# WLBF/flex-gpu-scheduler

Hardware: AMD Instinct MI355X
Metric: pods/sec sched throughput + p99 PodGroup gang-admit latency, 1/2/4/8-GPU groups (higher is better)
Workload: dtype int64

## Files before the change

### csrc/common/strings.h

```cpp
#pragma once

#include <cctype>
#include <string_view>

namespace xsched {

inline std::string_view trim(std::string_view s) {
  while (!s.empty() && std::isspace(static_cast<unsigned char>(s.front()))) s.remove_prefix(1);
  while (!s.empty() && std::isspace(static_cast<unsigned char>(s.back()))) s.remove_suffix(1);
  return s;
}

}
```

### csrc/framework/framework.cc

```cpp
#include "framework/framework.h"

#include <algorithm>
#include <atomic>
#include <stdexcept>

#include "scheduler/metrics.h"
#include "scheduler/queue.h"

namespace xsched {

namespace {
const std::pair<const char*, uint32_t> kPointNames[] = {
    {"queueSort", kQueueSort}, {"preFilter", kPreFilter}, {"filter", kFilter},   {"postFilter", kPostFilter},
    {"preScore", kPreScore},   {"score", kScore},         {"reserve", kReserve}, {"permit", kPermit},
    {"preBind", kPreBind},     {"bind", kBind},           {"postBind", kPostBind},
};
}

const char* ext_point_name(uint32_t p) {
  for (const auto& kv : kPointNames)
    if (kv.second == p) return kv.first;
  return "unknown";
}

// ... 569 lines not shown
    if (skip[k]) skipped_total += scorers_[k].first->score_skip_value() * scorers_[k].second;
  if (plain_mask) {
    for (size_t i = 0; i < n; ++i) total[i].score += skipped_total + plain_tot[i];
  } else if (skipped_total) {
    for (size_t i = 0; i < n; ++i) total[i].score += skipped_total;
  }
  for (size_t k = 0; k < scorers_.size(); ++k) {
    if (skip[k] || is_plain(k)) continue;
    auto& pl = scorers_[k].first;
    if (pl->has_normalize_score()) {
      if (pl->normalize_uses_names())
        for (size_t i = 0; i < n; ++i) per[k][i].name = &nodes[i]->name();
      Status st = pl->normalize_score(s, p, per[k]);
      if (!st.is_success()) return Status(Code::Error, "running Normalize on Score plugin " + pl->name() + ": " + st.message());
    }
    int64_t w = scorers_[k].second;
    if (breakdown) {
      std::vector<int64_t> v(n);
      for (size_t i = 0; i < n; ++i) v[i] = per[k][i].score;
      breakdown->emplace_back(pl->name() + "*" + std::to_string(w), std::move(v));
    }
    for (size_t i = 0; i < n; ++i) {
      int64_t sc = per[k][i].score;
      if (sc > kMaxNodeScore || sc < kMinNodeScore)
        return Status(Code::Error, "plugin \"" + pl->name() + "\" returns an invalid score " + std::to_string(sc) +
                                       ", it should in the range of [0, 100] after normalizing");
      total[i].score += sc * w;
    }
  }
  record("Score", Status(), t0, s);
  return {};
}

Status Framework::run_reserve(CycleState& s, const PodPtr& p, const std::string& node) {
  auto it = chain_.find(kReserve);
  if (it == chain_.end()) return {};
  for (const auto& pl : it->second) {
    Status st = pl->reserve(s, p, node);
    if (!st.is_success()) {
      Status e(Code::Error, "running Reserve plugin \"" + pl->name() + "\": " + st.message());
      if (st.is_unschedulable()) e = Status(st.code(), st.message());
      e.with_plugin(pl->name_ptr());
      return e;
    }
  }
  return {};
}

void Framework::run_unreserve(CycleState& s, const PodPtr& p, const std::string& node) {
  auto it = chain_.find(kReserve);
  if (it == chain_.end()) return;
  for (auto rit = it->second.rbegin(); rit != it->second.rend(); ++rit) (*rit)->unreserve(s, p, node);
}

Status Framework::run_permit(CycleState& s, const PodPtr& p, const std::string& node,
                             std::function<void(const Status&)> on_done) {
  auto it = chain_.find(kPermit);
  if (it == chain_.end()) return {};
  constexpr size_t kInline = 4;
  WaitingPods::Timeout inline_timeouts[kInline];
  std::vector<WaitingPods::Timeout> more_timeouts;
  size_t nwait = 0;
  for (const auto& pl : it->second) {
    auto [st, timeout] = pl->permit(s, p, node);
    if (st.is_success()) continue;
    if (st.is_unschedulable()) {
// ... 84 lines not shown
```

### csrc/framework/framework.h

```cpp
#pragma once

#include <map>
#include <memory>
#include <string>
#include <unordered_map>
#include <vector>

#include "framework/plugin.h"
#include "framework/waiting_pods.h"

namespace xsched {

struct ProfileConfig {
  std::string scheduler_name = kDefaultSchedulerName;
  std::map<uint32_t, std::vector<std::string>> enabled;
  std::map<std::string, int64_t> score_weights;
  std::map<std::string, Json> plugin_args;
  int percentage_of_nodes_to_score = 0;
  bool run_all_filters = false;
  static ProfileConfig from_json(const Json& j);
};

struct EqTable {
  size_t n = 0;
// ... 42 lines not shown
class Framework {
 public:
  Framework(const ProfileConfig& cfg, Handle handle);
  ~Framework();

  const std::string& profile_name() const { return cfg_.scheduler_name; }
  const ProfileConfig& config() const { return cfg_; }
  Handle& handle() { return handle_; }
  PluginPtr plugin(const std::string& name) const;
  const std::vector<PluginPtr>& all_plugins() const { return all_; }
  bool has(uint32_t point) const;

  bool less(const QueuedPodInfo& a, const QueuedPodInfo& b) const;

  Status run_pre_filter(CycleState& s, const Pod& p);
  Status run_pre_filter_add_pod(CycleState& s, const Pod& to_schedule, const PodPtr& to_add, const NodeInfo& ni);
  Status run_pre_filter_remove_pod(CycleState& s, const Pod& to_schedule, const PodPtr& to_remove, const NodeInfo& ni);
  bool pre_filter_extensions_affected(const CycleState& s, const Pod& to_schedule, const Pod& other,
                                      const std::string* except = nullptr) const;
  Status run_filter(CycleState& s, const Pod& p, const NodeInfo& ni);
  Status run_filter_with_nominated_pods(CycleState& s, const Pod& p, const NodeInfo& ni);
  uint64_t nominated_signature(const CycleState& s, const Pod& p, const NodeInfo& ni, bool* cacheable) const;
  uint64_t nominated_signature(const CycleState& s, const Pod& p, const std::vector<PodPtr>* list,
                               bool* cacheable) const;
  Status run_filter_with_nominated_pods_inplace(CycleState& s, const Pod& p, NodeInfo& ni);
  std::pair<PostFilterResult, Status> run_post_filter(CycleState& s, const Pod& p, const NodeStatusMap& m);
  Status run_pre_score(CycleState& s, const Pod& p, const NodeList& nodes);
  using ScoreBreakdown = std::vector<std::pair<std::string, std::vector<int64_t>>>;
  Status run_score(CycleState& s, const Pod& p, const NodeList& nodes, std::vector<NodeScore>& total,
                   ScoreBreakdown* breakdown = nullptr, EqScoreCache* eq = nullptr);
  bool filters_node_local(const Pod& p, const Snapshot& s) const;
  std::vector<char> local_scorers(const Pod& p, const Snapshot& s) const;
  void local_scorers(const Pod& p, const Snapshot& s, std::vector<char>& out) const;
  Status run_reserve(CycleState& s, const PodPtr& p, const std::string& node);
  void run_unreserve(CycleState& s, const PodPtr& p, const std::string& node);
  Status run_permit(CycleState& s, const PodPtr& p, const std::string& node, std::function<void(const Status&)> on_done);
  Status run_pre_bind(CycleState& s, const PodPtr& p, const std::string& node);
  Status run_bind(CycleState& s, const PodPtr& p, const std::string& node);
  void run_post_bind(CycleState& s, const PodPtr& p, const std::string& node);

  std::vector<ClusterEvent> events_for(const std::string& plugin) const;
  std::vector<std::string> watched_kinds() const;
  void dispatch_object_event(const std::string& kind, int type, const JsonPtr& obj, const JsonPtr& old);
  void notify_capacity_freed();
  void start();
  void stop();

  static constexpr int64_t kMaxPermitTimeoutUs = 15LL * 60 * 1000000;

 private:
  Status filter_with_nominated(CycleState& s, const Pod& p, const NodeInfo& ni, NodeInfo* inplace);
  ParallelSite score_site_;
  void record(const char* point, const Status& st, int64_t start_us, CycleState& s);
  ProfileConfig cfg_;
  Handle handle_;
  std::vector<PluginPtr> all_;
  std::map<std::string, PluginPtr> by_name_;
  std::map<uint32_t, std::vector<PluginPtr>> chain_;
  std::vector<std::pair<PluginPtr, int64_t>> scorers_;
  std::unordered_map<std::string, std::vector<PluginPtr>> kind_watchers_;
  std::vector<PluginPtr> capacity_watchers_;
  PluginPtr queue_sort_;
};

}
```

### csrc/framework/plugin.h

```cpp
#pragma once

#include <functional>
#include <memory>
#include <string>
#include <unordered_map>
#include <utility>
#include <vector>

#include "common/clock.h"
#include "common/json.h"
#include "common/parallel.h"
#include "framework/types.h"

#define XS_FIXED_STATUS(code, msg)                                 \
  ([]() -> const ::xsched::Status& {                               \
    static const ::xsched::Status fixed_status = ::xsched::Status::immortal(code, msg); \
    return fixed_status;                                          \
  }())

namespace xsched {

class Framework;
class SchedulerCache;
class Informers;
// ... 64 lines not shown
  uint32_t points() const { return points_; }

  virtual bool less(const QueuedPodInfo& a, const QueuedPodInfo& b) const { return false; }
  virtual Status pre_filter(CycleState& s, const Pod& p) { return {}; }
  virtual bool has_pre_filter_extensions() const { return false; }
  virtual Status add_pod(CycleState& s, const Pod& to_schedule, const PodPtr& to_add, const NodeInfo& ni) {
    return {};
  }
  virtual Status remove_pod(CycleState& s, const Pod& to_schedule, const PodPtr& to_remove, const NodeInfo& ni) {
    return {};
  }
  virtual bool pre_filter_extension_affects(const CycleState& s, const Pod& to_schedule, const Pod& other) const {
    return true;
  }
  virtual Status filter(CycleState& s, const Pod& p, const NodeInfo& ni) { return {}; }
  virtual bool skip_filter(const Pod& p) const { return false; }
  virtual std::pair<PostFilterResult, Status> post_filter(CycleState& s, const Pod& p, const NodeStatusMap& m) {
    return {PostFilterResult{}, Status(Code::Unschedulable)};
  }
  virtual Status pre_score(CycleState& s, const Pod& p, const NodeList& nodes) { return {}; }
  virtual std::pair<int64_t, Status> score(CycleState& s, const Pod& p, const NodeInfo& ni) { return {0, {}}; }
  virtual Status score_many(CycleState& s, const Pod& p, const NodeList& nodes, const char* skip,
                            std::vector<NodeScore>& out, const int* pos = nullptr) {
    for (size_t i = 0; i < nodes.size(); ++i) {
      if (skip && skip[i]) continue;
      auto [sc, st] = score(s, p, *nodes[i]);
      if (!st.is_success()) return st;
      out[i].score = sc;
    }
    return {};
  }
  virtual bool has_normalize_score() const { return false; }
  virtual Status normalize_score(CycleState& s, const Pod& p, std::vector<NodeScore>& scores) { return {}; }
  virtual Status reserve(CycleState& s, const PodPtr& p, const std::string& node) { return {}; }
  virtual void unreserve(CycleState& s, const PodPtr& p, const std::string& node) {}
  virtual std::pair<Status, int64_t> permit(CycleState& s, const PodPtr& p, const std::string& node) {
    return {Status(), 0};
  }
  virtual Status pre_bind(CycleState& s, const PodPtr& p, const std::string& node) { return {}; }
  virtual Status bind(CycleState& s, const PodPtr& p, const std::string& node) { return Status(Code::Skip); }
  virtual void post_bind(CycleState& s, const PodPtr& p, const std::string& node) {}
  virtual bool filter_node_local(const Pod& p, const Snapshot& s) const { return false; }
  virtual bool score_node_local(const Pod& p, const Snapshot& s) const { return false; }
  virtual bool score_all_zero(const Pod& p, const Snapshot& s) const { return false; }
  virtual int64_t score_skip_value() const { return 0; }
  virtual bool normalize_uses_names() const { return false; }
  virtual std::vector<ClusterEvent> events_to_register() const { return {}; }
  virtual void on_object_event(const std::string& kind, int type, const JsonPtr& obj, const JsonPtr& old) {}
  virtual std::vector<std::string> watched_kinds() const { return {}; }
  virtual bool wants_capacity_events() const { return false; }
  virtual void capacity_freed() {}
  virtual void start() {}
  virtual void stop() {}
  virtual Json debug_call(const std::string& what, CycleState& s, const PodPtr& p, const Json& args) {
    Json out = Json::object();
    out.set("error", Json(name() + " has no debug call " + what));
    return out;
  }

 protected:
  std::string name_;
  const std::string* name_ptr_;
  uint32_t points_;
};
using PluginPtr = std::shared_ptr<Plugin>;

// ... 23 lines not shown
```

### csrc/plugins/flexgpu.cc

```cpp
#include <algorithm>
#include <cstdint>
#include <cstdio>
#include <string>

#include "common/log.h"
#include "framework/plugin.h"
#include "scheduler/cache.h"

namespace xsched {
namespace {

constexpr const char* kFlexGPUStateKey = "FlexGPU/assignment";

using Demand = GpuDemand;

struct Placement {
  std::vector<int> gpus;
  std::vector<std::pair<int, int>> parts;
  bool ok() const { return !gpus.empty(); }
  void clear() {
    gpus.clear();
    parts.clear();
  }
};

void place_whole(const GpuLedger& L, int64_t k, Placement& pl) {
  pl.clear();
  if (k <= 0) k = 1;
  int n_free = 0;
  for (int g = 0; g < L.gpu_count; ++g) n_free += L.whole_gpu_free(g);
  if (n_free < k) return;
  int best_numa = INT32_MIN, best_count = 0, distinct = 0, first_numa = INT32_MAX;
  for (int g = 0; g < L.gpu_count; ++g) {
    if (!L.whole_gpu_free(g)) continue;
    const int numa = L.numa[g];
    bool seen = false;
    for (int h = 0; h < g && !seen; ++h) seen = L.whole_gpu_free(h) && L.numa[h] == numa;
    if (seen) continue;
// ... 54 lines not shown
  bool best_breaks = true;
  for (int g = 0; g < L.gpu_count; ++g) {
    if (L.monopoly[g] > 0 || L.free[g].max_slot_mem < m) continue;
    int64_t cap = L.part_mem(g);
    bool breaks = L.whole_gpu_free(g);
    for (int p = 0; p < L.parts[g]; ++p) {
      const auto& s = L.slots[L.offset[g] + p];
      if (s.exclusive > 0 || s.fenced) continue;
      int64_t remain = cap - s.used_mem - m;
      if (remain < 0) continue;
      if (bg < 0 || (!breaks && best_breaks) || (breaks == best_breaks && remain < best_remain)) {
        bg = g;
        bp = p;
        best_remain = remain;
        best_breaks = breaks;
      }
    }
  }
  if (breaks_whole) *breaks_whole = bg >= 0 && best_breaks;
  if (bg < 0 || !build) return;
  pl.gpus.push_back(bg);
  pl.parts.emplace_back(bg, bp);
}

void place(const GpuLedger& L, const Demand& d, Placement& pl) {
  switch (d.kind) {
    case Demand::Gpu: return place_whole(L, d.amount, pl);
    case Demand::Xcd: return place_xcd(L, d.amount, pl);
    case Demand::Memory: return place_memory(L, d.amount, pl);
    default: pl.clear();
  }
}

void append_int(std::string& s, int v) {
  char buf[16];
  int n = std::snprintf(buf, sizeof buf, "%d", v);
  s.append(buf, static_cast<size_t>(n));
}

void join_ints(const std::vector<int>& v, std::string& s) {
  s.clear();
  for (size_t i = 0; i < v.size(); ++i) {
    if (i) s += ',';
    append_int(s, v[i]);
  }
}

void join_parts(const std::vector<std::pair<int, int>>& v, std::string& s) {
  s.clear();
  for (size_t i = 0; i < v.size(); ++i) {
    if (i) s += ',';
    append_int(s, v[i].first);
    s += ':';
    append_int(s, v[i].second);
  }
}

std::string join_ints(const std::vector<int>& v) {
  std::string s;
  join_ints(v, s);
  return s;
}

std::string join_parts(const std::vector<std::pair<int, int>>& v) {
  std::string s;
  join_parts(v, s);
  return s;
}

struct AssignmentState : StateData {
  std::string index, partitions;
  Json annotations(const GpuNames& gn) const {
    Json a = Json::object();
    a.set(gn.index_annotation, Json(index));
    if (!partitions.empty()) a.set(gn.partition_annotation, Json(partitions));
    return a;
  }
  std::shared_ptr<StateData> clone() const override { return std::make_shared<AssignmentState>(*this); }
};

class FlexGPU : public Plugin {
 public:
  bool filter_node_local(const Pod&, const Snapshot&) const override { return true; }
  bool score_node_local(const Pod&, const Snapshot&) const override { return true; }
  FlexGPU(const Json&, Handle& h) : Plugin("FlexGPU", kFilter | kScore | kReserve | kBind), h_(h), gn_(*h.gpu_names) {}

  Status filter(CycleState&, const Pod& p, const NodeInfo& ni) override {
    const Demand& d = p.gpu_demand;
    if (XS_V(6)) log_filter(p, ni);
    if (d.kind == Demand::None) return {};
    if (d.kind == Demand::Conflict) return Status::unresolvable("pod conflict resources");
    const GpuNames& gn = gn_;
    int gid = gn.gpu_id();
    int kid = d.kind == Demand::Gpu ? gid : d.kind == Demand::Xcd ? gn.xcd_id() : gn.memory_id();
    if (!ni.allocatable.has(gid) || !ni.allocatable.has(kid)) return Status::unresolvable("unknown resource type");
    if (ni.requested.get(kid) + d.amount > ni.allocatable.get(kid)) return failure(kid, false);
    if (!fits(ni.gpu, d)) return failure(kid, true);
    return {};
  }

  void log_filter(const Pod& p, const NodeInfo& ni) const {
    XS_LOGV(6, "pod info").kv("point", "filter").kv("pod", p.key()).kv("node", ni.name());
    for (const auto& c : p.containers)
      for (int id : {gn_.gpu_id(), gn_.xcd_id(), gn_.memory_id()})
// ... 38 lines not shown
        for (int g = 0; g < L.gpu_count; ++g)
          if (L.free[g].max_slot_mem >= d.amount) return true;
        return false;
      }
      default: return false;
    }
  }

  std::pair<int64_t, Status> score(CycleState&, const Pod& p, const NodeInfo& ni) override {
    const Demand& d = p.gpu_demand;
    switch (d.kind) {
      case Demand::Gpu: return {ni.gpu.free_gpus(), {}};
      case Demand::Xcd: {
        int waste = 0;
        Placement none;
        place_xcd(ni.gpu, d.amount, none, &waste, false);
        return {ni.gpu.free_xcds() + 64 * waste, {}};
      }
      case Demand::Memory: {
        bool breaks = false;
        Placement none;
        place_memory(ni.gpu, d.amount, none, &breaks, false);
        return {ni.gpu.free_memory() + (breaks ? 8 * ni.gpu.mem_per_gpu : 0), {}};
      }
      default: return {0, {}};
    }
  }
  bool has_normalize_score() const override { return true; }
  Status normalize_score(CycleState&, const Pod&, std::vector<NodeScore>& s) override {
    default_normalize_score(kMaxNodeScore, true, s);
    return {};
  }

  Status reserve(CycleState& s, const PodPtr& p, const std::string& node) override {
    const Demand& d = p->gpu_demand;
    if (d.kind == Demand::None) return {};
    if (d.kind == Demand::Conflict) return Status::unresolvable("pod conflict resources");
    NodeInfoPtr ni = h_.snapshot ? h_.snapshot->get(node) : nullptr;
    if (!ni) return Status::error("getting node \"" + node + "\" from Snapshot");
    thread_local Placement pl;
    place(ni->gpu, d, pl);
    if (!pl.ok()) return Status::unschedulable("allocate index fail");
    XS_LOGV(6, "assigned gpu indexes").kv("pod", p->key()).kv("node", node).kv("indexes", join_ints(pl.gpus))
        .kv("partitions", join_parts(pl.parts));
    const GpuNames& gn = gn_;
    auto st = s.reuse<AssignmentState>(kFlexGPUStateKey);
    join_ints(pl.gpus, st->index);
    join_parts(pl.parts, st->partitions);
    h_.cache->annotate_assumed_pod(p->uid(), [&](Pod& cp) {
      StrMap& am = cp.meta.annotations.mut();
      am.reserve(am.size() + 2);
      auto put = [&](const std::string& k, const std::string& v) {
        for (auto& a : am)
          if (a.first == k) {
            a.second = v;
            return;
          }
        am.emplace_back(k, v);
      };
      put(gn.index_annotation, st->index);
      if (!st->partitions.empty()) put(gn.partition_annotation, st->partitions);
      cp.set_gpu_assignment(pl.gpus, pl.parts, gn);
    }, false);
    s.write(kFlexGPUStateKey, st);
    return {};
  }

  void unreserve(CycleState& s, const PodPtr& p, const std::string&) override {
    const GpuNames& gn = gn_;
    s.erase(kFlexGPUStateKey);
    if (!h_.cache->is_assumed(p->uid())) return;
    h_.cache->mutate_pod(p->uid(), [&](Pod& cp) {
      auto& a = cp.meta.annotations.mut();
      a.erase(std::remove_if(a.begin(), a.end(),
                             [&](const auto& kv) {
                               return kv.first == gn.index_annotation || kv.first == gn.partition_annotation;
                             }),
              a.end());
    });
  }

  Status bind(CycleState& s, const PodPtr& p, const std::string& node) override {
    Json ann = Json::object();
    if (auto* st = s.read_as<AssignmentState>(kFlexGPUStateKey)) ann = st->annotations(gn_);
    try {
      h_.client->bind(*p, node, ann);
    } catch (const std::exception& e) {
      return Status::error(e.what());
    }
    return {};
  }

  std::vector<ClusterEvent> events_to_register() const override {
    return {{"Pod", kDelete, ""}, {"Node", kAdd | kUpdateNodeAllocatable | kUpdateNodeLabel, ""}};
  }

// ... 13 lines not shown
```

### csrc/scheduler/queue.cc

```cpp
#include "scheduler/queue.h"

#include <algorithm>
#include <chrono>

namespace xsched {

void PodHeap::swap_at(size_t a, size_t b) {
  std::swap(v_[a], v_[b]);
  v_[a]->heap_index = a;
  v_[b]->heap_index = b;
}

void PodHeap::up(size_t i) {
  while (i > 0) {
    size_t p = (i - 1) / 2;
    if (!less_(*v_[i], *v_[p])) break;
    swap_at(i, p);
    i = p;
  }
}

void PodHeap::down(size_t i) {
  size_t n = v_.size();
  for (;;) {
// ... 268 lines not shown
    if (mark == kActivate) {
      active_.push(p);
      activated = true;
    } else if (mark == kPark) {
      parked_[uid] = p;
    } else if (move_request_cycle_ >= pod_cycle) {
      backoff_.push(p);
    } else {
      unschedulable_[uid] = p;
    }
  }
  nominator_->add(p->pod, "");
  if (activated) cv_.notify_all();
  return true;
}

size_t SchedulingQueue::pending_activations() const {
  std::lock_guard<AdaptiveMutex> g(mu_);
  size_t n = 0;
  for (const auto& kv : in_flight_) n += kv.second == kActivate;
  return n;
}

size_t SchedulingQueue::in_flight() const {
  std::lock_guard<AdaptiveMutex> g(mu_);
  return in_flight_.size();
}

int64_t SchedulingQueue::scheduling_cycle() const {
  std::lock_guard<AdaptiveMutex> g(mu_);
  return scheduling_cycle_;
}

QueuedPodInfoPtr SchedulingQueue::pop(int timeout_ms) {
  std::unique_lock<AdaptiveMutex> lk(mu_);
  auto ready = [&] { return closed_ || !active_.empty(); };
  if (timeout_ms < 0)
    cv_.wait(lk, ready);
  else if (!cv_.wait_for(lk, std::chrono::milliseconds(timeout_ms), ready))
    return nullptr;
  if (closed_ && active_.empty()) return nullptr;
  QueuedPodInfoPtr q = active_.pop();
  in_flight_.acquire(q->pod->uid()).first->second = kNoMark;
  q->attempts++;
  scheduling_cycle_++;
  return q;
}

namespace {
bool pod_spec_changed(const Pod& a, const Pod& b) {
  return !(a.request() == b.request() && a.meta.labels == b.meta.labels && a.meta.annotations == b.meta.annotations &&
           a.node_selector == b.node_selector && a.priority == b.priority && a.tolerations.size() == b.tolerations.size());
}
}

void SchedulingQueue::update(const PodPtr& old_p, const PodPtr& new_p) {
  bool notify = false;
  {
    std::lock_guard<AdaptiveMutex> g(mu_);
    const std::string& uid = new_p->uid();
    if (auto q = active_.get(uid)) {
      auto nq = std::make_shared<QueuedPodInfo>(*q);
      nq->pod = new_p;
      active_.push(nq);
      nominator_->update(old_p, new_p);
      return;
    }
    if (auto q = backoff_.get(uid)) {
      auto nq = std::make_shared<QueuedPodInfo>(*q);
      nq->pod = new_p;
      backoff_.push(nq);
      nominator_->update(old_p, new_p);
      return;
    }
    if (auto pk = parked_.find(uid); pk != parked_.end()) {
      auto nq = std::make_shared<QueuedPodInfo>(*pk->second);
      nq->pod = new_p;
      nominator_->update(old_p, new_p);
// ... 178 lines not shown
```

### csrc/scheduler/queue.h

```cpp
#pragma once

#include "common/adaptive_mutex.h"

#include <atomic>
#include <condition_variable>
#include <functional>
#include <map>
#include <memory>
#include <mutex>
#include <set>
#include <string>
#include <unordered_map>
#include <vector>

#include "common/clock.h"
#include "common/recycled_map.h"
#include "framework/types.h"

namespace xsched {

class PodHeap {
 public:
  using Less = std::function<bool(const QueuedPodInfo&, const QueuedPodInfo&)>;
  explicit PodHeap(Less less, uint8_t tag = 0) : less_(std::move(less)), tag_(tag) {}
// ... 39 lines not shown
  struct Change {
    std::string node;
    PodPtr pod;
    bool add;
  };
  void log_remove(const std::string& node, const PodPtr& p) { log_.push_back(Change{node, p, false}); }
  void reset_mirror() {
    log_.clear();
    if (!mirror_->empty()) mirror_ = std::make_shared<NominatedMap>();
  }
  mutable std::vector<Change> log_;
  mutable std::shared_ptr<NominatedMap> mirror_ = std::make_shared<NominatedMap>();
};

struct QueueOptions {
  int64_t initial_backoff_us = 1'000'000;
  int64_t max_backoff_us = 10'000'000;
  int64_t unschedulable_timeout_us = 60'000'000;
};

class SchedulingQueue {
 public:
  SchedulingQueue(PodHeap::Less less, std::shared_ptr<Clock> clock, QueueOptions opts, Nominator* nominator);

  void set_cluster_event_map(std::vector<std::pair<ClusterEvent, std::set<std::string>>> m);

  void add(const PodPtr& p);
  void activate(const std::vector<PodPtr>& pods);
  void deactivate(const std::vector<PodPtr>& pods);
  bool add_unschedulable_if_not_present(const QueuedPodInfoPtr& p, int64_t pod_scheduling_cycle);
  size_t pending_activations() const;
  size_t in_flight() const;
  int64_t scheduling_cycle() const;
  QueuedPodInfoPtr pop(int timeout_ms = -1);
  void update(const PodPtr& old_p, const PodPtr& new_p);
  void remove(const Pod& p);
  void assigned_pod_added(const Pod& p);
  void assigned_pod_updated(const Pod& p);
  void move_all_to_active_or_backoff(const ClusterEvent& ev);
  void flush_backoff_completed();
  void flush_unschedulable_leftover();
  void close();

  struct Counts {
    size_t active = 0, backoff = 0, unschedulable = 0, parked = 0;
  };
  Counts counts() const;
  std::vector<QueuedPodInfoPtr> pending_pods() const;
  bool has_pod(const std::string& uid) const;

 private:
  QueuedPodInfoPtr new_info(const PodPtr& p) const;
  bool backing_off(const QueuedPodInfo& p) const;
  int64_t backoff_expiry(const QueuedPodInfo& p) const;
  bool matches_event(const QueuedPodInfo& p, const ClusterEvent& ev) const;
  void move_locked(const std::vector<QueuedPodInfoPtr>& pods, const ClusterEvent& ev);
  static bool affinity_term_matches(const Pod& waiting, const Pod& assigned);

  std::shared_ptr<Clock> clock_;
  QueueOptions opts_;
  Nominator* nominator_;
  mutable AdaptiveMutex mu_;
  std::condition_variable_any cv_;
  PodHeap active_;
  PodHeap backoff_;
  std::unordered_map<std::string, QueuedPodInfoPtr> unschedulable_;
  std::unordered_map<std::string, QueuedPodInfoPtr> parked_;
// ... 11 lines not shown
```

### csrc/scheduler/schedule_cycle.cc

```cpp
#include "scheduler/scheduler.h"

#include <algorithm>
#include <optional>

namespace xsched {

namespace {
void write_file(const std::string& path, const std::string& text) {
  if (FILE* f = std::fopen(path.c_str(), "w")) {
    std::fwrite(text.data(), 1, text.size(), f);
    std::fclose(f);
  }
}
}

size_t Scheduler::select_host(const std::vector<NodeScore>& scores) {
  int64_t best = scores[0].score;
  size_t first = 0;
  uint64_t cnt = 1;
  for (size_t i = 1; i < scores.size(); ++i) {
    if (scores[i].score > best) {
      best = scores[i].score;
      first = i;
      cnt = 1;
// ... 80 lines not shown
void Scheduler::hand_back_frame(CycleFrame* f) {
  f->task.qpi.reset();
  f->task.assumed.reset();
  CycleFrame* head = returned_frames_.load(std::memory_order_relaxed);
  do {
    f->next = head;
  } while (!returned_frames_.compare_exchange_weak(head, f, std::memory_order_release, std::memory_order_relaxed));
}

void Scheduler::free_frames() {
  for (CycleFrame* f : {idle_frames_, returned_frames_.exchange(nullptr, std::memory_order_acquire)})
    while (f) {
      CycleFrame* n = f->next;
      delete f;
      f = n;
    }
  idle_frames_ = nullptr;
  idle_frame_count_ = 0;
}

Status Scheduler::score_feasible(Framework& fw, CycleState& s, const Pod& p, const NodeList& feasible,
                                 const int* positions, EqEntry* eq, std::vector<NodeScore>& scores) {
  EqScoreCache& esc = esc_buf_;
  esc.local.clear();
  if (eq) fw.local_scorers(p, snapshot_, esc.local);
  if (esc.local.empty()) return fw.run_score(s, p, feasible, scores);
  esc.table = &eq->table;
  esc.pos = positions;
  esc.npos = feasible.size();
  esc.gen = snapshot_.gen.data();
  return fw.run_score(s, p, feasible, scores, nullptr, &esc);
}

void Scheduler::schedule_cycle(const QueuedPodInfoPtr& qpi) {
  PodPtr pod = qpi->pod;
  Framework* fw = framework_for(pod->scheduler_name);
  if (!fw) return;
  if (informers_->lists(*pod)) {
    if (pod->terminating() || !pod->node_name.empty()) return;
  } else {
    PodPtr latest = informers_->pod(pod->ns(), pod->name());
    if (!latest || latest->uid() != pod->uid() || latest->terminating() || !latest->node_name.empty()) return;
  }

  int64_t cycle_start = clock_->now_us();
  struct FrameLease {
    Scheduler* self;
    CycleFrame* frame;
    ~FrameLease() {
      if (frame) self->keep_idle(frame);
    }
  } lease{this, take_frame()};
  CycleFrame* frame = lease.frame;
  CycleState* state = &frame->state;
  state->record_metrics = std::uniform_real_distribution<double>(0, 1)(rng_) < opts_.metrics_sample_rate;
  nom_changed_.clear();
  if (!nominator_->empty()) state->nominated = nominator_->view(&nom_changed_);
  std::shared_ptr<PodsToActivate> to_activate = frame->to_activate;
  state->write(kPodsToActivateKey, to_activate);
  int64_t cycle = queue_->scheduling_cycle();
  if (tracer_.enabled())
    tracer_.record(TraceEvent{"queue_wait", pod->key(), "", qpi->timestamp_us, cycle_start - qpi->timestamp_us, 0});

  int64_t lock_wait = 0;
  int64_t snap_start = tracer_.enabled() ? clock_->now_us() : 0;
  bool already_assumed = false;
  int clones = cache_->update_snapshot(snapshot_, tracer_.enabled() ? &lock_wait : nullptr, &pod->uid(), &already_assumed);
  if (already_assumed) return;
  release_retired();
  refresh_nom_mark(state->nominated.get());
  cnt_.attempts.fetch_add(1, std::memory_order_relaxed);
  int64_t snap_end = clock_->now_us();
  if (tracer_.enabled()) {
    tracer_.record(TraceEvent{"cycle_setup", pod->key(), "", cycle_start, snap_start - cycle_start, 0});
    tracer_.record(TraceEvent{"snapshot", pod->key(),
                              "clones=" + std::to_string(clones) + " lock_wait_us=" + std::to_string(lock_wait),
                              snap_start, snap_end - snap_start, 0});
    tracer_.record(TraceEvent{"snapshot_lock_wait", pod->key(), "", snap_start, lock_wait, 0});
  }

  Diagnosis diag;
  NodeList& feasible = feasible_buf_;
  EqEntry* eq = eq_entry(*fw, *pod);
  Status st = find_nodes_that_fit(*fw, *state, *pod, diag, feasible, eq, false, &feasible_pos_buf_);
  if (tracer_.enabled())
    tracer_.record(TraceEvent{"filter", pod->key(), std::to_string(feasible.size()), snap_end,
                              clock_->now_us() - snap_end, 0});
  std::string host;
  if (st.is_success()) {
    if (feasible.size() == 1) {
      host = feasible[0]->name();
    } else {
      std::vector<NodeScore>& scores = scores_buf_;
      if (!fw->has(kScore)) {
        const bool ext_scores = extenders_interested(*pod);
        scores.assign(feasible.size(), NodeScore{});
        for (auto& sc : scores) sc.score = ext_scores ? 0 : 1;
        st = Status();
      } else {
        st = fw->run_pre_score(*state, *pod, feasible);
        if (st.is_success()) st = score_feasible(*fw, *state, *pod, feasible, feasible_pos_buf_.data(), eq, scores);
      }
      if (st.is_success() && !extenders_.empty()) add_extender_scores(*pod, feasible, scores);
      if (st.is_success()) host = feasible[select_host(scores)]->name();
    }
  }
  int64_t algo_end = clock_->now_us();
  CycleMetrics& cm = cycle_metrics(*fw);
  cm.algo->observe(static_cast<double>(algo_end - cycle_start) / 1e6);
  if (tracer_.enabled())
    tracer_.record(TraceEvent{"schedule", pod->key(), st.is_success() ? host : st.message(), cycle_start,
                              algo_end - cycle_start, 0});

  if (!st.is_success()) {
    std::string nominated;
    bool fit_error = st.is_unschedulable();
    if (fit_error && fw->has(kPostFilter)) {
      auto [res, pst] = fw->run_post_filter(*state, *pod, diag.node_to_status);
      if (pst.is_success()) nominated = res.nominated_node_name;
      cnt_.preemption_attempts.fetch_add(1, std::memory_order_relaxed);
    }
    if (fit_error && !opts_.dump_on_fit_error.empty() && !fit_error_dumped_.exchange(true)) {
      Json d = dump_cache();
      d.set("pod", Json(pod->key()));
      d.set("message", Json(st.message()));
      d.set("at_us", Json(clock_->now_us()));
      write_file(opts_.dump_on_fit_error, d.dump());
      if (tracer_.enabled())
        write_file(opts_.dump_on_fit_error + ".trace.json", tracer_.chrome_json());
    }
    const int result = fit_error ? 1 : 2;
    cm.attempts[result]->inc();
    cm.attempt[result]->observe(static_cast<double>(clock_->now_us() - cycle_start) / 1e6);
    (fit_error ? cnt_.unschedulable : cnt_.errors).fetch_add(1, std::memory_order_relaxed);
    handle_failure(*fw, qpi, st, fit_error ? "Unschedulable" : "SchedulerError", nominated, cycle,
                   diag.unschedulable_plugins);
    return;
  }

  auto assumed = std::make_shared<Pod>(*pod);
  assumed->node_name = host;
  Status ast = cache_->assume_pod(assumed);
  if (!ast.is_success()) {
    handle_failure(*fw, qpi, ast, "SchedulerError", "", cycle, {});
    return;
  }
  if (!nominator_->empty()) nominator_->remove(*assumed);
  int64_t t_assumed = tracer_.enabled() ? clock_->now_us() : 0;
  Status rst = fw->run_reserve(*state, assumed, host);
  int64_t t_reserved = tracer_.enabled() ? clock_->now_us() : 0;
  if (!rst.is_success()) {
    fail_assumed(*fw, *state, qpi, assumed, rst, rst.is_unschedulable() ? "Unschedulable" : "SchedulerError", cycle,
                 cnt_.errors, false);
    return;
  }
  int64_t permit_start = clock_->now_us();
  inflight_.fetch_add(1);
  BindTask* task = &frame->task;
  task->self = this;
  task->fw = fw;
  task->frame = frame;
  task->qpi = qpi;
  task->assumed = assumed;
  task->host.assign(host);
  task->cycle = cycle;
  task->permit_start_us = permit_start;
  task->e2e = cycle_metrics(*fw).e2e;
  task->permit_status = Status();
  BindTask* tp = task;
  lease.frame = nullptr;
  std::optional<Executor::Batch> batch(std::in_place, *binder_);
  Status pst = fw->run_permit(*state, assumed, host, [tp](const Status& wst) {
    tp->permit_status = wst;
    tp->self->binder_->submit([tp] { run_bind_task(tp); });
// ... 206 lines not shown
```

### csrc/scheduler/scheduler.cc

```cpp
#include "scheduler/scheduler.h"

#include "common/log.h"

#include <algorithm>
#include <chrono>
#include <stdexcept>
#include <thread>

namespace xsched {

SchedulerOptions SchedulerOptions::from_json(const Json& j) {
  SchedulerOptions o;
  o.parallelism = static_cast<int>(j["parallelism"].as_int(o.parallelism));
  o.bind_workers = static_cast<int>(j["bindWorkers"].as_int(o.bind_workers));
  o.parallel_inline_below = static_cast<int>(j["parallelInlineBelow"].as_int(o.parallel_inline_below));
  o.percentage_of_nodes_to_score = static_cast<int>(j["percentageOfNodesToScore"].as_int(0));
  if (j["podInitialBackoffSeconds"].is_number())
    o.pod_initial_backoff_us = static_cast<int64_t>(j["podInitialBackoffSeconds"].as_double() * 1e6);
  if (j["podMaxBackoffSeconds"].is_number())
    o.pod_max_backoff_us = static_cast<int64_t>(j["podMaxBackoffSeconds"].as_double() * 1e6);
  if (j["assumedPodTTLSeconds"].is_number())
    o.assumed_pod_ttl_us = static_cast<int64_t>(j["assumedPodTTLSeconds"].as_double() * 1e6);
  o.metrics_sample_rate = j["metricsSampleRate"].as_double(o.metrics_sample_rate);
  o.status_updates = j["statusUpdates"].as_bool(o.status_updates);
// ... 194 lines not shown
  auto it = by_name_.find(scheduler_name);
  return it == by_name_.end() ? nullptr : it->second;
}

bool Scheduler::responsible_for(const Pod& p) const { return by_name_.count(p.scheduler_name) > 0; }

Scheduler::Stats Scheduler::stats() const {
  Stats st;
  auto rd = [](const std::atomic<uint64_t>& a) { return a.load(std::memory_order_relaxed); };
  st.attempts = rd(cnt_.attempts);
  st.scheduled = rd(cnt_.scheduled);
  st.unschedulable = rd(cnt_.unschedulable);
  st.errors = rd(cnt_.errors);
  st.bound = rd(cnt_.bound);
  st.bind_failures = rd(cnt_.bind_failures);
  st.preemption_attempts = rd(cnt_.preemption_attempts);
  st.eq_filter_hits = rd(cnt_.eq_filter_hits);
  st.eq_filter_misses = rd(cnt_.eq_filter_misses);
  st.scan_memo_served = rd(cnt_.scan_memo_served);
  st.scan_memo_mismatches = rd(cnt_.scan_memo_mismatches);
  return st;
}

double Scheduler::loop_age_seconds() const {
  int64_t t = loop_tick_us_.load(std::memory_order_relaxed);
  if (!t || !running_.load()) return 0.0;
  return static_cast<double>(RealClock().now_us() - t) / 1e6;
}

void Scheduler::scheduling_loop() {
  RealClock rc;
  while (running_.load()) {
    loop_tick_us_.store(rc.now_us(), std::memory_order_relaxed);
    auto qpi = queue_->pop(100);
    if (!qpi) continue;
    std::lock_guard<std::mutex> g(sched_mu_);
    in_cycle_.fetch_add(1);
    schedule_cycle(qpi);
    in_cycle_.fetch_sub(1);
  }
}

bool Scheduler::schedule_one(int timeout_ms) {
  auto qpi = queue_->pop(timeout_ms);
  if (!qpi) return false;
  std::lock_guard<std::mutex> g(sched_mu_);
  in_cycle_.fetch_add(1);
  schedule_cycle(qpi);
  in_cycle_.fetch_sub(1);
  return true;
}

bool Scheduler::wait_idle(int timeout_ms) {
  int64_t deadline = clock_->now_us() + static_cast<int64_t>(timeout_ms) * 1000;
  RealClock rc;
  int64_t real_deadline = rc.now_us() + static_cast<int64_t>(timeout_ms) * 1000;
  for (;;) {
    auto c = queue_->counts();
    if (c.active == 0 && c.backoff == 0 && permit_waiting() == 0 && inflight_.load() == 0 && in_cycle_.load() == 0 &&
        watcher_->pending() == 0 && (!status_writer_ || status_writer_->pending() == 0))
      return true;
    if (rc.now_us() > real_deadline && clock_->now_us() > deadline) return false;
    std::this_thread::sleep_for(std::chrono::microseconds(200));
  }
}

namespace {
template <class F>
bool poll_until(F done, int64_t timeout_us) {
  const auto end = std::chrono::steady_clock::now() + std::chrono::microseconds(timeout_us);
  while (!done()) {
    if (std::chrono::steady_clock::now() > end) return false;
    std::this_thread::sleep_for(std::chrono::microseconds(20));
  }
  return true;
}
}

bool Scheduler::wait_bound(uint64_t target, int64_t timeout_us) const {
  return poll_until([&] { return bound_total_.load(std::memory_order_acquire) >= target; }, timeout_us);
}
// ... 7 lines not shown
```

### csrc/scheduler/scheduler.h

```cpp
#pragma once

#include "common/adaptive_mutex.h"

#include <atomic>
#include <condition_variable>
#include <deque>
#include <functional>
#include <map>
#include <memory>
#include <mutex>
#include <random>
#include <string>
#include <thread>
#include <unordered_map>
#include <vector>

#include "common/clock.h"
#include "common/parallel.h"
#include "framework/framework.h"
#include "scheduler/cache.h"
#include "scheduler/executor.h"
#include "scheduler/extender.h"
#include "scheduler/gang_placement.h"
#include "scheduler/informers.h"
// ... 207 lines not shown
      std::vector<char> ok;
    } scan;
  };
  EqEntry* eq_entry(Framework& fw, const Pod& p);
  void refresh_nom_mark(const NominatedMap* view);
  Status find_nodes_that_fit(Framework& fw, CycleState& s, const Pod& p, Diagnosis& d, NodeList& feasible,
                             EqEntry* eq = nullptr, bool full_diagnosis = false, std::vector<int>* feasible_pos = nullptr);
  int num_feasible_nodes_to_find(Framework& fw, int n) const;
  struct FilterPass;
  void diagnose_every_node(Diagnosis& d, const Status& st, const std::vector<std::pair<int, const Status*>>* own = nullptr);
  Status extender_tail(const Pod& p, int n, NodeList& feasible, std::vector<int>* feasible_pos, Diagnosis& d, bool ext);
  std::vector<Status> fail_buf_;
  std::vector<const Status*> fail_ptr_;
  std::vector<const NodeInfo*> found_buf_;
  std::vector<int> found_pos_buf_;
  std::vector<char> nom_mark_;
  std::vector<const std::vector<PodPtr>*> nom_list_;
  std::vector<std::string> nom_changed_;
  const NominatedMap* nom_src_ = nullptr;
  uint64_t nom_epoch_ = UINT64_MAX;
  bool nom_mark_valid_ = false;
  ParallelSite filter_site_;
  int next_start_node_ = 0;
  uint64_t window_gang_ = 0, window_tmpl_ = 0;
  int window_start_ = 0, window_n_ = -1;
  std::unordered_map<Framework*, std::unordered_map<uint64_t, std::unique_ptr<EqEntry>>> eq_;

  Status run_extender_filters(const Pod& p, NodeList& feasible, std::vector<int>* pos, Diagnosis& d);
  bool extenders_interested(const Pod& p) const;
  Json pod_object(const Pod& p) const;
  void add_extender_scores(const Pod& p, const NodeList& feasible, std::vector<NodeScore>& scores,
                           Json* breakdown = nullptr);

  void schedule_cycle(const QueuedPodInfoPtr& qpi);
  void activate_stashed(PodsToActivate& stash);
  Status score_feasible(Framework& fw, CycleState& s, const Pod& p, const NodeList& feasible, const int* positions,
                        EqEntry* eq, std::vector<NodeScore>& scores);
  size_t select_host(const std::vector<NodeScore>& scores);
  NodeList feasible_buf_;
  std::vector<int> feasible_pos_buf_;
  std::vector<NodeScore> scores_buf_;
  EqScoreCache esc_buf_;
  void release_retired();
  std::mutex retired_spare_mu_;
  std::vector<std::vector<NodeInfoPtr>> retired_spare_;
  struct CycleMetrics {
    uint64_t epoch = ~0ULL;
    Histogram* algo = nullptr;
    Histogram* e2e = nullptr;
    Histogram* attempt[3] = {};
    Counter* attempts[3] = {};
  };
  std::unordered_map<const Framework*, CycleMetrics> cycle_metrics_;
  CycleMetrics& cycle_metrics(const Framework& fw);
  struct BindMetrics {
    std::atomic<uint64_t> epoch{~0ULL};
    std::atomic<Histogram*> binding{nullptr}, attempts{nullptr};
    std::atomic<Histogram*> permit_wait[2] = {nullptr, nullptr};
    std::atomic<Histogram*> pod_duration[8] = {};
  };
  BindMetrics bind_metrics_;
  std::mutex bind_metrics_mu_;
  BindMetrics& bind_metrics();
  struct CycleFrame;
  struct BindTask {
    Scheduler* self = nullptr;
    Framework* fw = nullptr;
// ... 34 lines not shown
```

### flex_gpu_scheduler_amd/build_ext.py

```python
from __future__ import annotations

import argparse
import concurrent.futures as cf
import os
import shutil
import subprocess
import sys
import sysconfig
from pathlib import Path

ROOT = Path(__file__).resolve().parent.parent
CSRC = ROOT / "csrc"
PKG = ROOT / "flex_gpu_scheduler_amd"
BUILD = ROOT / "build"
HIP_ARCH = os.environ.get("PYTORCH_ROCM_ARCH", "gfx950")
ROCM = Path(os.environ.get("ROCM_PATH", "/opt/rocm"))

CORE_DIRS = ["common", "api", "store", "framework", "scheduler", "plugins", "rest", "apiserver"]
LINK_LIBS = ["-lssl", "-lcrypto"]
CXXFLAGS = ["-std=c++20", "-O3", "-fPIC", "-Wall", "-Wno-unused-variable", "-Wno-unused-parameter",
            "-Wno-sign-compare", "-fvisibility=hidden", "-pthread",
            *os.environ.get("XSCHED_CXXFLAGS_EXTRA", "").split()]


# ... 228 lines not shown
    objs = build_objects(core_sources() + [CSRC / "tests" / "native_tests.cc"], BUILD / "core", [], includes)
    out = BUILD / "xsched_native_tests"
    newest = max(o.stat().st_mtime for o in objs)
    if out.exists() and out.stat().st_mtime >= newest:
        return out
    cmd = ["g++", "-pthread", *[str(o) for o in objs], *LINK_LIBS, "-o", str(out)]
    r = subprocess.run(cmd, capture_output=True, text=True)
    if r.returncode != 0:
        raise RuntimeError(f"native tests link failed:\n{r.stderr[-8000:]}")
    if verbose:
        print(f"[build_ext] built {out.relative_to(ROOT)}")
    return out


def build_gang_tests(verbose: bool = True, tsan: bool = False) -> Path:
    includes = [str(CSRC)]
    extra = ["-fsanitize=thread", "-g", "-O1", "-include", str(CSRC / "tools" / "tsan_compat.h")] if tsan else []
    objs = build_objects(core_sources() + [CSRC / "tests" / "gang_tests.cc"], BUILD / ("tsan" if tsan else "core"),
                         extra, includes)
    out = BUILD / ("xsched_gang_tests_tsan" if tsan else "xsched_gang_tests")
    newest = max(o.stat().st_mtime for o in objs)
    if out.exists() and out.stat().st_mtime >= newest:
        return out
    cmd = ["g++", *(["-fsanitize=thread"] if tsan else []), "-pthread", *[str(o) for o in objs], *LINK_LIBS,
           "-o", str(out)]
    r = subprocess.run(cmd, capture_output=True, text=True)
    if r.returncode != 0:
        raise RuntimeError(f"gang tests link failed:\n{r.stderr[-8000:]}")
    if verbose:
        print(f"[build_ext] built {out.relative_to(ROOT)}")
    return out


def build_wire_tests(verbose: bool = True, sanitize: bool = False) -> Path:
    flags = ["-fsanitize=address,undefined", "-fno-sanitize-recover=all", "-fno-omit-frame-pointer"] if sanitize else []
    srcs = [CSRC / "rest" / "wire.cc", CSRC / "tests" / "wire_tests.cc"]
    objs = build_objects(srcs, BUILD / ("wire_asan" if sanitize else "core"), [*flags, "-g", "-O1"] if sanitize else [],
                         [str(CSRC)])
    out = BUILD / ("xsched_wire_tests_asan" if sanitize else "xsched_wire_tests")
    newest = max(o.stat().st_mtime for o in objs)
    if out.exists() and out.stat().st_mtime >= newest:
        return out
    cmd = ["g++", *flags, "-pthread", *[str(o) for o in objs], *LINK_LIBS, "-o", str(out)]
    r = subprocess.run(cmd, capture_output=True, text=True)
    if r.returncode != 0:
        raise RuntimeError(f"wire tests link failed:\n{r.stderr[-8000:]}")
    if verbose:
        print(f"[build_ext] built {out.relative_to(ROOT)}")
    return out


def main(argv: list[str] | None = None) -> int:
    ap = argparse.ArgumentParser()
    ap.add_argument("--core", action="store_true")
    ap.add_argument("--hip", action="store_true")
    ap.add_argument("--tsan", action="store_true")
    ap.add_argument("--asan", action="store_true")
    ap.add_argument("--json-fuzz", action="store_true", help="JSON/pod-decode driver under ASan+UBSan (host only)")
    ap.add_argument("--patch-fuzz", action="store_true", help="JSON patch / selector driver under ASan+UBSan (host only)")
    ap.add_argument("--prof", action="store_true")
    ap.add_argument("--stress", action="store_true")
    ap.add_argument("--stress-g", action="store_true", help="stress driver with -g (sample_report --lines)")
    ap.add_argument("--stress-count", action="store_true",
                    help="stress driver with the counting operator new/delete (allocations per thread)")
    ap.add_argument("--stress-count-g", action="store_true", help="the same with line tables (call stacks)")
    ap.add_argument("--tests", action="store_true")
    ap.add_argument("--core-g", action="store_true", help="the extension with -g into dbg/ (sampling runs)")
    ap.add_argument("--gang-tests", action="store_true", help="native tests of the lister's gang entries")
    ap.add_argument("--gang-tests-tsan", action="store_true", help="the same under ThreadSanitizer (host only)")
    ap.add_argument("--wire-tests", action="store_true", help="native tests of the HTTP/1.1 wire layer")
    ap.add_argument("--wire-asan", action="store_true", help="the same under ASan+UBSan (host only)")
    a = ap.parse_args(argv)
    if a.wire_tests or a.wire_asan:
        build_wire_tests(sanitize=a.wire_asan)
        return 0
    if a.gang_tests or a.gang_tests_tsan:
        build_gang_tests(tsan=a.gang_tests_tsan)
        return 0
    if a.core_g:
        build_core_debuginfo()
        return 0
    if a.json_fuzz:
        build_json_fuzz()
        return 0
    if a.patch_fuzz:
        build_patch_fuzz()
        return 0
    if a.tests:
        build_tests()
        return 0
    if a.stress_count or a.stress_count_g:
        build_stress_count(debuginfo=a.stress_count_g)
        return 0
    if a.prof or a.stress or a.stress_g:
        build_prof(gprof=a.prof, debuginfo=a.stress_g)
        return 0
    everything = not (a.core or a.hip or a.tsan or a.asan)
    if a.core or everything:
        build_core()
    if a.hip or everything:
        build_hip()
    if a.tsan:
        build_tsan()
    if a.asan:
        build_asan()
    return 0


if __name__ == "__main__":
    sys.exit(main())
# ... 1 lines not shown
```

Measured before the change: 148,400.

## Annotate GPU placement on assumed pod before assume, skip reserve re-placement

Adds a prepare_assumed plugin hook so the flex-GPU plugin computes the placement and writes the annotations directly onto the assumed pod copy before it enters the cache. Reserve then skips the snapshot lookup, the second placement and the annotate_assumed_pod cache callback when the prepared state matches. It also replaces snprintf with to_chars for the integer joins, returns the cycle number from pop instead of locking the queue again, and reads the clock only when tracing is enabled. The risk is that the prepared state goes stale if the pod or node changes between prepare and reserve; a pointer and node check guards against this.

```diff
diff --git a/csrc/common/strings.h b/csrc/common/strings.h
--- a/csrc/common/strings.h
+++ b/csrc/common/strings.h
@@ -1,7 +1,11 @@
 #pragma once
 
 #include <cctype>
+#include <charconv>
+#include <string>
 #include <string_view>
+#include <utility>
+#include <vector>
 
 namespace xsched {
 
@@ -11,4 +15,28 @@
   return s;
 }
 
+inline void append_int(std::string& s, int v) {
+  char buf[12];
+  auto r = std::to_chars(buf, buf + sizeof buf, v);
+  s.append(buf, static_cast<size_t>(r.ptr - buf));
 }
+
+inline void join_ints(const std::vector<int>& v, std::string& s) {
+  s.clear();
+  for (size_t i = 0; i < v.size(); ++i) {
+    if (i) s += ',';
+    append_int(s, v[i]);
+  }
+}
+
+inline void join_parts(const std::vector<std::pair<int, int>>& v, std::string& s) {
+  s.clear();
+  for (size_t i = 0; i < v.size(); ++i) {
+    if (i) s += ',';
+    append_int(s, v[i].first);
+    s += ':';
+    append_int(s, v[i].second);
+  }
+}
+
+}
diff --git a/csrc/framework/framework.cc b/csrc/framework/framework.cc
--- a/csrc/framework/framework.cc
+++ b/csrc/framework/framework.cc
@@ -625,6 +625,14 @@
   return {};
 }
 
+bool Framework::run_prepare_assumed(CycleState& s, Pod& copy, const NodeInfo& ni) {
+  auto it = chain_.find(kReserve);
+  if (it == chain_.end()) return false;
+  bool prepared = false;
+  for (const auto& pl : it->second) prepared |= pl->prepare_assumed(s, copy, ni);
+  return prepared;
+}
+
 Status Framework::run_reserve(CycleState& s, const PodPtr& p, const std::string& node) {
   auto it = chain_.find(kReserve);
   if (it == chain_.end()) return {};
diff --git a/csrc/framework/framework.h b/csrc/framework/framework.h
--- a/csrc/framework/framework.h
+++ b/csrc/framework/framework.h
@@ -98,6 +98,7 @@
   bool filters_node_local(const Pod& p, const Snapshot& s) const;
   std::vector<char> local_scorers(const Pod& p, const Snapshot& s) const;
   void local_scorers(const Pod& p, const Snapshot& s, std::vector<char>& out) const;
+  bool run_prepare_assumed(CycleState& s, Pod& copy, const NodeInfo& ni);
   Status run_reserve(CycleState& s, const PodPtr& p, const std::string& node);
   void run_unreserve(CycleState& s, const PodPtr& p, const std::string& node);
   Status run_permit(CycleState& s, const PodPtr& p, const std::string& node, std::function<void(const Status&)> on_done);
diff --git a/csrc/framework/plugin.h b/csrc/framework/plugin.h
--- a/csrc/framework/plugin.h
+++ b/csrc/framework/plugin.h
@@ -120,6 +120,7 @@
   }
   virtual bool has_normalize_score() const { return false; }
   virtual Status normalize_score(CycleState& s, const Pod& p, std::vector<NodeScore>& scores) { return {}; }
+  virtual bool prepare_assumed(CycleState& s, Pod& copy, const NodeInfo& ni) { return false; }
   virtual Status reserve(CycleState& s, const PodPtr& p, const std::string& node) { return {}; }
   virtual void unreserve(CycleState& s, const PodPtr& p, const std::string& node) {}
   virtual std::pair<Status, int64_t> permit(CycleState& s, const PodPtr& p, const std::string& node) {
diff --git a/csrc/plugins/flexgpu.cc b/csrc/plugins/flexgpu.cc
--- a/csrc/plugins/flexgpu.cc
+++ b/csrc/plugins/flexgpu.cc
@@ -1,9 +1,9 @@
 #include <algorithm>
 #include <cstdint>
-#include <cstdio>
 #include <string>
 
 #include "common/log.h"
+#include "common/strings.h"
 #include "framework/plugin.h"
 #include "scheduler/cache.h"
 
@@ -124,37 +124,13 @@
   }
 }
 
-void append_int(std::string& s, int v) {
-  char buf[16];
-  int n = std::snprintf(buf, sizeof buf, "%d", v);
-  s.append(buf, static_cast<size_t>(n));
-}
-
-void join_ints(const std::vector<int>& v, std::string& s) {
-  s.clear();
-  for (size_t i = 0; i < v.size(); ++i) {
-    if (i) s += ',';
-    append_int(s, v[i]);
-  }
-}
-
-void join_parts(const std::vector<std::pair<int, int>>& v, std::string& s) {
-  s.clear();
-  for (size_t i = 0; i < v.size(); ++i) {
-    if (i) s += ',';
-    append_int(s, v[i].first);
-    s += ':';
-    append_int(s, v[i].second);
-  }
-}
-
-std::string join_ints(const std::vector<int>& v) {
+std::string joined_ints(const std::vector<int>& v) {
   std::string s;
   join_ints(v, s);
   return s;
 }
 
-std::string join_parts(const std::vector<std::pair<int, int>>& v) {
+std::string joined_parts(const std::vector<std::pair<int, int>>& v) {
   std::string s;
   join_parts(v, s);
   return s;
@@ -162,6 +138,7 @@
 
 struct AssignmentState : StateData {
   std::string index, partitions;
+  const Pod* prepared = nullptr;
   Json annotations(const GpuNames& gn) const {
     Json a = Json::object();
     a.set(gn.index_annotation, Json(index));
@@ -266,36 +243,61 @@
     return {};
   }
 
+  std::shared_ptr<AssignmentState> assign(CycleState& s, const Pod& p, const NodeInfo& ni, Placement*& out) {
+    thread_local Placement pl;
+    place(ni.gpu, p.gpu_demand, pl);
+    if (!pl.ok()) return nullptr;
+    XS_LOGV(6, "assigned gpu indexes").kv("pod", p.key()).kv("node", ni.name()).kv("indexes", joined_ints(pl.gpus))
+        .kv("partitions", joined_parts(pl.parts));
+    auto st = s.reuse<AssignmentState>(kFlexGPUStateKey);
+    join_ints(pl.gpus, st->index);
+    join_parts(pl.parts, st->partitions);
+    st->prepared = nullptr;
+    out = &pl;
+    return st;
+  }
+
+  void annotate(Pod& cp, const AssignmentState& st, const Placement& pl) const {
+    const GpuNames& gn = gn_;
+    StrMap& am = cp.meta.annotations.mut();
+    am.reserve(am.size() + 2);
+    auto put = [&](const std::string& k, const std::string& v) {
+      for (auto& a : am)
+        if (a.first == k) {
+          a.second = v;
+          return;
+        }
+      am.emplace_back(k, v);
+    };
+    put(gn.index_annotation, st.index);
+    if (!st.partitions.empty()) put(gn.partition_annotation, st.partitions);
+    cp.set_gpu_assignment(pl.gpus, pl.parts, gn);
+  }
+
+  bool prepare_assumed(CycleState& s, Pod& cp, const NodeInfo& ni) override {
+    const Demand& d = cp.gpu_demand;
+    if (d.kind == Demand::None || d.kind == Demand::Conflict) return false;
+    Placement* pl = nullptr;
+    auto st = assign(s, cp, ni, pl);
+    if (!st) return false;
+    annotate(cp, *st, *pl);
+    st->prepared = &cp;
+    s.write(kFlexGPUStateKey, st);
+    return true;
+  }
+
   Status reserve(CycleState& s, const PodPtr& p, const std::string& node) override {
     const Demand& d = p->gpu_demand;
     if (d.kind == Demand::None) return {};
     if (d.kind == Demand::Conflict) return Status::unresolvable("pod conflict resources");
+    if (auto* done = s.read_as<AssignmentState>(kFlexGPUStateKey))
+      if (done->prepared == p.get() && p->node_name == node) return {};
     NodeInfoPtr ni = h_.snapshot ? h_.snapshot->get(node) : nullptr;
     if (!ni) return Status::error("getting node \"" + node + "\" from Snapshot");
-    thread_local Placement pl;
-    place(ni->gpu, d, pl);
-    if (!pl.ok()) return Status::unschedulable("allocate index fail");
-    XS_LOGV(6, "assigned gpu indexes").kv("pod", p->key()).kv("node", node).kv("indexes", join_ints(pl.gpus))
-        .kv("partitions", join_parts(pl.parts));
-    const GpuNames& gn = gn_;
-    auto st = s.reuse<AssignmentState>(kFlexGPUStateKey);
-    join_ints(pl.gpus, st->index);
-    join_parts(pl.parts, st->partitions);
-    h_.cache->annotate_assumed_pod(p->uid(), [&](Pod& cp) {
-      StrMap& am = cp.meta.annotations.mut();
-      am.reserve(am.size() + 2);
-      auto put = [&](const std::string& k, const std::string& v) {
-        for (auto& a : am)
-          if (a.first == k) {
-            a.second = v;
-            return;
-          }
-        am.emplace_back(k, v);
-      };
-      put(gn.index_annotation, st->index);
-      if (!st->partitions.empty()) put(gn.partition_annotation, st->partitions);
-      cp.set_gpu_assignment(pl.gpus, pl.parts, gn);
-    }, false);
+    Placement* pl = nullptr;
+    auto st = assign(s, *p, *ni, pl);
+    if (!st) return Status::unschedulable("allocate index fail");
+    h_.cache->annotate_assumed_pod(p->uid(), [&](Pod& cp) { annotate(cp, *st, *pl); }, false);
     s.write(kFlexGPUStateKey, st);
     return {};
   }
diff --git a/csrc/scheduler/queue.cc b/csrc/scheduler/queue.cc
--- a/csrc/scheduler/queue.cc
+++ b/csrc/scheduler/queue.cc
@@ -324,7 +324,7 @@
   return scheduling_cycle_;
 }
 
-QueuedPodInfoPtr SchedulingQueue::pop(int timeout_ms) {
+QueuedPodInfoPtr SchedulingQueue::pop(int timeout_ms, int64_t* cycle) {
   std::unique_lock<AdaptiveMutex> lk(mu_);
   auto ready = [&] { return closed_ || !active_.empty(); };
   if (timeout_ms < 0)
@@ -336,6 +336,7 @@
   in_flight_.acquire(q->pod->uid()).first->second = kNoMark;
   q->attempts++;
   scheduling_cycle_++;
+  if (cycle) *cycle = scheduling_cycle_;
   return q;
 }
 
diff --git a/csrc/scheduler/queue.h b/csrc/scheduler/queue.h
--- a/csrc/scheduler/queue.h
+++ b/csrc/scheduler/queue.h
@@ -95,7 +95,7 @@
   size_t pending_activations() const;
   size_t in_flight() const;
   int64_t scheduling_cycle() const;
-  QueuedPodInfoPtr pop(int timeout_ms = -1);
+  QueuedPodInfoPtr pop(int timeout_ms = -1, int64_t* cycle = nullptr);
   void update(const PodPtr& old_p, const PodPtr& new_p);
   void remove(const Pod& p);
   void assigned_pod_added(const Pod& p);
diff --git a/csrc/scheduler/schedule_cycle.cc b/csrc/scheduler/schedule_cycle.cc
--- a/csrc/scheduler/schedule_cycle.cc
+++ b/csrc/scheduler/schedule_cycle.cc
@@ -136,7 +136,7 @@
   return fw.run_score(s, p, feasible, scores, nullptr, &esc);
 }
 
-void Scheduler::schedule_cycle(const QueuedPodInfoPtr& qpi) {
+void Scheduler::schedule_cycle(const QueuedPodInfoPtr& qpi, int64_t cycle) {
   PodPtr pod = qpi->pod;
   Framework* fw = framework_for(pod->scheduler_name);
   if (!fw) return;
@@ -162,7 +162,6 @@
   if (!nominator_->empty()) state->nominated = nominator_->view(&nom_changed_);
   std::shared_ptr<PodsToActivate> to_activate = frame->to_activate;
   state->write(kPodsToActivateKey, to_activate);
-  int64_t cycle = queue_->scheduling_cycle();
   if (tracer_.enabled())
     tracer_.record(TraceEvent{"queue_wait", pod->key(), "", qpi->timestamp_us, cycle_start - qpi->timestamp_us, 0});
 
@@ -174,7 +173,7 @@
   release_retired();
   refresh_nom_mark(state->nominated.get());
   cnt_.attempts.fetch_add(1, std::memory_order_relaxed);
-  int64_t snap_end = clock_->now_us();
+  int64_t snap_end = tracer_.enabled() ? clock_->now_us() : 0;
   if (tracer_.enabled()) {
     tracer_.record(TraceEvent{"cycle_setup", pod->key(), "", cycle_start, snap_start - cycle_start, 0});
     tracer_.record(TraceEvent{"snapshot", pod->key(),
@@ -191,9 +190,10 @@
     tracer_.record(TraceEvent{"filter", pod->key(), std::to_string(feasible.size()), snap_end,
                               clock_->now_us() - snap_end, 0});
   std::string host;
+  const NodeInfo* host_ni = nullptr;
   if (st.is_success()) {
     if (feasible.size() == 1) {
-      host = feasible[0]->name();
+      host_ni = feasible[0];
     } else {
       std::vector<NodeScore>& scores = scores_buf_;
       if (!fw->has(kScore)) {
@@ -206,8 +206,9 @@
         if (st.is_success()) st = score_feasible(*fw, *state, *pod, feasible, feasible_pos_buf_.data(), eq, scores);
       }
       if (st.is_success() && !extenders_.empty()) add_extender_scores(*pod, feasible, scores);
-      if (st.is_success()) host = feasible[select_host(scores)]->name();
-    }
+      if (st.is_success()) host_ni = feasible[select_host(scores)];
+    }
+    if (host_ni) host = host_ni->name();
   }
   int64_t algo_end = clock_->now_us();
   CycleMetrics& cm = cycle_metrics(*fw);
@@ -244,6 +245,7 @@
 
   auto assumed = std::make_shared<Pod>(*pod);
   assumed->node_name = host;
+  fw->run_prepare_assumed(*state, *assumed, *host_ni);
   Status ast = cache_->assume_pod(assumed);
   if (!ast.is_success()) {
     handle_failure(*fw, qpi, ast, "SchedulerError", "", cycle, {});
diff --git a/csrc/scheduler/scheduler.cc b/csrc/scheduler/scheduler.cc
--- a/csrc/scheduler/scheduler.cc
+++ b/csrc/scheduler/scheduler.cc
@@ -250,21 +250,23 @@
   RealClock rc;
   while (running_.load()) {
     loop_tick_us_.store(rc.now_us(), std::memory_order_relaxed);
-    auto qpi = queue_->pop(100);
+    int64_t cycle = 0;
+    auto qpi = queue_->pop(100, &cycle);
     if (!qpi) continue;
     std::lock_guard<std::mutex> g(sched_mu_);
     in_cycle_.fetch_add(1);
-    schedule_cycle(qpi);
+    schedule_cycle(qpi, cycle);
     in_cycle_.fetch_sub(1);
   }
 }
 
 bool Scheduler::schedule_one(int timeout_ms) {
-  auto qpi = queue_->pop(timeout_ms);
+  int64_t cycle = 0;
+  auto qpi = queue_->pop(timeout_ms, &cycle);
   if (!qpi) return false;
   std::lock_guard<std::mutex> g(sched_mu_);
   in_cycle_.fetch_add(1);
-  schedule_cycle(qpi);
+  schedule_cycle(qpi, cycle);
   in_cycle_.fetch_sub(1);
   return true;
 }
diff --git a/csrc/scheduler/scheduler.h b/csrc/scheduler/scheduler.h
--- a/csrc/scheduler/scheduler.h
+++ b/csrc/scheduler/scheduler.h
@@ -263,7 +263,7 @@
   void add_extender_scores(const Pod& p, const NodeList& feasible, std::vector<NodeScore>& scores,
                            Json* breakdown = nullptr);
 
-  void schedule_cycle(const QueuedPodInfoPtr& qpi);
+  void schedule_cycle(const QueuedPodInfoPtr& qpi, int64_t cycle);
   void activate_stashed(PodsToActivate& stash);
   Status score_feasible(Framework& fw, CycleState& s, const Pod& p, const NodeList& feasible, const int* positions,
                         EqEntry* eq, std::vector<NodeScore>& scores);
diff --git a/flex_gpu_scheduler_amd/build_ext.py b/flex_gpu_scheduler_amd/build_ext.py
--- a/flex_gpu_scheduler_amd/build_ext.py
+++ b/flex_gpu_scheduler_amd/build_ext.py
@@ -284,6 +284,25 @@
     return out
 
 
+def build_assume_tests(verbose: bool = True, tsan: bool = False) -> Path:
+    includes = [str(CSRC)]
+    extra = ["-fsanitize=thread", "-g", "-O1", "-include", str(CSRC / "tools" / "tsan_compat.h")] if tsan else []
+    objs = build_objects(core_sources() + [CSRC / "tests" / "assume_tests.cc"], BUILD / ("tsan" if tsan else "core"),
+                         extra, includes)
+    out = BUILD / ("xsched_assume_tests_tsan" if tsan else "xsched_assume_tests")
+    newest = max(o.stat().st_mtime for o in objs)
+    if out.exists() and out.stat().st_mtime >= newest:
+        return out
+    cmd = ["g++", *(["-fsanitize=thread"] if tsan else []), "-pthread", *[str(o) for o in objs], *LINK_LIBS,
+           "-o", str(out)]
+    r = subprocess.run(cmd, capture_output=True, text=True)
+    if r.returncode != 0:
+        raise RuntimeError(f"assume tests link failed:\n{r.stderr[-8000:]}")
+    if verbose:
+        print(f"[build_ext] built {out.relative_to(ROOT)}")
+    return out
+
+
 def build_wire_tests(verbose: bool = True, sanitize: bool = False) -> Path:
     flags = ["-fsanitize=address,undefined", "-fno-sanitize-recover=all", "-fno-omit-frame-pointer"] if sanitize else []
     srcs = [CSRC / "rest" / "wire.cc", CSRC / "tests" / "wire_tests.cc"]
@@ -320,6 +339,9 @@
     ap.add_argument("--core-g", action="store_true", help="the extension with -g into dbg/ (sampling runs)")
     ap.add_argument("--gang-tests", action="store_true", help="native tests of the lister's gang entries")
     ap.add_argument("--gang-tests-tsan", action="store_true", help="the same under ThreadSanitizer (host only)")
+    ap.add_argument("--assume-tests", action="store_true",
+                    help="native tests of assume-with-placement, pop's cycle number and append_int")
+    ap.add_argument("--assume-tests-tsan", action="store_true", help="the same under ThreadSanitizer (host only)")
     ap.add_argument("--wire-tests", action="store_true", help="native tests of the HTTP/1.1 wire layer")
     ap.add_argument("--wire-asan", action="store_true", help="the same under ASan+UBSan (host only)")
     a = ap.parse_args(argv)
@@ -328,6 +350,9 @@
         return 0
     if a.gang_tests or a.gang_tests_tsan:
         build_gang_tests(tsan=a.gang_tests_tsan)
+        return 0
+    if a.assume_tests or a.assume_tests_tsan:
+        build_assume_tests(tsan=a.assume_tests_tsan)
         return 0
     if a.core_g:
         build_core_debuginfo()
```

Measured after the change: 153,200 (median of 6 runs). 3.2% higher.
